# luisdiaz1997/GPzoo

Hardware: AMD Instinct MI355X
Metric: ELBO evals/sec (L=32-latent evaluations, all GPUs) at M=2048 inducing, N=200000, L=32 latents/GPU x 1 GPU(s) (higher is better)
Workload: dtype f32; 1 GPU; BASELINE configs[2]: Slide-seq-shaped synthetic, N=200000 spots, M=2048, L=32 latents/GPU x 1 GPU(s), matern32, f32; latents_total=32, whitened=True, chunk=0, factor_dtype=f64

## Files before the change

gpzoo_amd/_lib.py:

```python
from __future__ import annotations

import ctypes as C
import os

HERE = os.path.dirname(os.path.abspath(__file__))
LIB_PATH = os.environ.get("GPZ_HIP_LIB") or os.path.join(HERE, "libgpzoo_hip.so")

GPZ_F32, GPZ_F64 = 0, 1
KERNEL_RBF, KERNEL_MATERN32, KERNEL_MGGP_RBF, KERNEL_DISTANCE = 0, 1, 2, 3
KERNEL_MATERN12, KERNEL_MATERN52 = 4, 5
SVGP_MATERIALIZE_KZX, SVGP_NARROW_TILES, SVGP_GENERATE_KZX, SVGP_PANEL_PRODUCTS = 1, 2, 4, 8
SVGP_BACKWARD_ALGEBRA, SVGP_BACKWARD_CLASSIC = 16, 32
PROF_SLOTS = ("kfill", "stage1", "stage2", "potrf_trailing", "potrf_all", "trtri", "finalize", "_unused")


class KernelDesc(C.Structure):
    _fields_ = [
        ("kind", C.c_int32), ("n_latent", C.c_int32), ("dtype", C.c_int32), ("n_groups", C.c_int32),
        ("sigma", C.c_void_p), ("lengthscale", C.c_void_p), ("group_a", C.c_void_p), ("group_r2", C.c_void_p),
        ("group_pow", C.c_double),
    ]


class SvgpProblem(C.Structure):
    _fields_ = [
        ("k", KernelDesc),
        ("dtype", C.c_int32), ("whitened", C.c_int32), ("d", C.c_int32), ("flags", C.c_int32),
        ("N", C.c_int64), ("M", C.c_int64),
# ... 147 lines not shown
```

gpzoo_amd/build.py:

```python
from __future__ import annotations

import os
import subprocess
import sys

HERE = os.path.dirname(os.path.abspath(__file__))
CSRC = os.path.join(HERE, "csrc")
LIB = os.path.join(HERE, "libgpzoo_hip.so")
SOURCES = ["runtime.hip", "kfill.hip", "gemm.hip", "gemmw.hip", "gemmp.hip", "diag128.hip", "coop.hip", "factor.hip", "kgrad.hip", "mmops.hip", "poisson.hip", "svgp.hip", "vnngp.hip", "collective.hip", "spatial.hip", "nmf.hip", "smooth.hip", "kmeans.hip", "gram.hip", "poisson_sparse.hip"]
HEADERS = ["common.h", "gemm.h", "cov.h", "gemmw.h", "gemmp.h", "diag128.h", "factor.h", "kgrad.h", "mmops.h", os.path.join("..", "..", "include", "gpzoo_hip.h")]
FLAGS = ["--offload-arch=gfx950", "-O3", "-std=c++17", "-fPIC", "-ffp-contract=fast", "-Wall", "-Wno-unused-function"]
SOURCE_FLAGS = {"spatial.hip": ["-ffp-contract=off"], "smooth.hip": ["-ffp-contract=off"], "kmeans.hip": ["-ffp-contract=off"]}


HASH_MARK = b"GPZ_SRC_HASH:"


def source_hash():
    import hashlib
    h = hashlib.sha256()
    for f in sorted(SOURCES + HEADERS):
        path = os.path.join(CSRC, f)
        if not os.path.exists(path):
            return None
        h.update(os.path.basename(f).encode() + b"\0")
# ... 55 lines not shown
```

gpzoo_amd/csrc/common.h:

```cpp
#pragma once
#include <hip/hip_runtime.h>
#include <stdint.h>
#include <stddef.h>

#include "../../include/gpzoo_hip.h"

namespace gpz {

constexpr int PAD = 128;

inline int64_t pad_up(int64_t v, int64_t m = PAD) { return (v + m - 1) / m * m; }

void set_error(const char* fmt, ...);

#define GPZ_HIP_OK(expr)                                                          \
  do {                                                                            \
    hipError_t _e = (expr);                                                       \
    if (_e != hipSuccess) {                                                       \
      gpz::set_error("%s:%d: %s -> %s", __FILE__, __LINE__, #expr, hipGetErrorString(_e)); \
      return -2;                                                                  \
    }                                                                             \
  } while (0)

#define GPZ_REQUIRE(cond, ...)            \
// ... 14 lines not shown
  template <typename T>
  T* take(size_t count) {
    off = (off + 255) & ~size_t(255);
    T* r = base ? reinterpret_cast<T*>(base + off) : nullptr;
    off += count * sizeof(T);
    return r;
  }
  size_t used() const { return (off + 255) & ~size_t(255); }
};

int kfill_padded(const gpz_kernel_desc* k, const void* A, int64_t nA, int64_t pA, const void* B, int64_t nB,
                 int64_t pB, int d, const int64_t* gA, const int64_t* gB, void* K, int64_t ldk, int64_t stride,
                 double jitter, int pad_identity, int out_dtype, hipStream_t s, int32_t* bad_group = nullptr);

enum ProfSlot { PROF_KFILL = 0, PROF_STAGE1 = 1, PROF_STAGE2 = 2, PROF_POTRF_TRAIL = 3,
                PROF_POTRF_ALL = 4, PROF_TRTRI = 5, PROF_FINAL = 6, PROF_NSLOTS = 8 };
bool prof_enabled();
void prof_begin(int slot, hipStream_t s);
void prof_end(int slot, hipStream_t s);

}
```

gpzoo_amd/csrc/gemmp.h:

```cpp
#pragma once
#include "common.h"

namespace gpz {

struct PanelArgs {
  const float* Linv; const float* LuT;
  const float* Kzx;
  const float* Z; const float* X;
  const float* sigma; const float* ell;
  int64_t M, nreal; int kind, d;
  float* Wt;
  const float* muE;
  float* ps1; float* pm1; float* ps2;
  int64_t Mp, ncp; int L;
};
bool panel_supported(int64_t Mp, int64_t ncp);
bool panel_generates(int kind, int d);
int panel_launch(const PanelArgs& a, hipStream_t s);

}
```

gpzoo_amd/csrc/gemmp.hip:

```cpp
#include "gemmp.h"

#include "cov.h"

#include <cstdlib>
#include <mutex>
#include <type_traits>

#ifndef GPZ_P_ABL
#define GPZ_P_ABL 0
#endif

namespace gpz {

typedef float f32x4 __attribute__((ext_vector_type(4)));
typedef unsigned int u32x4 __attribute__((ext_vector_type(4)));

struct PanelParams {
  const float* Linv; const float* LuT;
  const float* Kzx;
  const float* Z; const float* X;
  const float* sigma; const float* ell;
  int M, nreal;
  float* Wt;
  const float* muE;
// ... 396 lines not shown
      case 6: return launch_t<NBV, 6>(p, store, s);          \
      case 7: return launch_t<NBV, 7>(p, store, s);          \
      case 8: return launch_t<NBV, 8>(p, store, s);          \
      default: return launch_t<NBV, 0>(p, store, s);         \
    }
  switch (a.Mp / 32) {
    GPZ_PANEL_CASE(4)
    GPZ_PANEL_CASE(8)
    GPZ_PANEL_CASE(12)
    default:
    GPZ_PANEL_CASE(16)
  }
#undef GPZ_PANEL_CASE
}

}

extern "C" void gpz_debug_panel_stamps(unsigned long long* buf) { gpz::g_panel_stamps = buf; }
```

gpzoo_amd/csrc/kgrad.hip:

```cpp
#include "kgrad.h"
#include "mmops.h"

namespace gpz {

__device__ __forceinline__ float kg_exp(float x) { return __builtin_amdgcn_exp2f(x * 1.44269504088896341f); }
__device__ __forceinline__ double kg_exp(double x) { return exp(x); }
__device__ __forceinline__ float kg_sqrt(float x) { return sqrtf(x); }
__device__ __forceinline__ double kg_sqrt(double x) { return sqrt(x); }
__device__ __forceinline__ float kg_rsqrt(float x) { return rsqrtf(x); }
__device__ __forceinline__ double kg_rsqrt(double x) { return 1.0 / sqrt(x); }
__device__ __forceinline__ float kg_pow(float x, float y) { return __builtin_amdgcn_exp2f(y * __builtin_amdgcn_logf(x)); }
__device__ __forceinline__ double kg_pow(double x, double y) { return pow(x, y); }

template <typename T, int KIND>
__global__ __launch_bounds__(256) void kgrad_kernel(KgradArgs a) {
  const int l = blockIdx.y, wave = threadIdx.x >> 6, lane = threadIdx.x & 63;
  const int64_t m = (int64_t)blockIdx.x * 4 + wave;
  if (m >= a.M) return;
  const T* kb = static_cast<const T*>(a.Kbar) + (int64_t)l * a.stride + m * a.ld;
  const T* Zp = static_cast<const T*>(a.Z);
  const T* Xp = static_cast<const T*>(a.X);
  const int d = a.d;
  const T sig = static_cast<const T*>(a.sigma)[l];
  const T ell = static_cast<const T*>(a.ell)[l];
  const T s2 = sig * sig, il2 = (T)1 / (ell * ell);
  T z[4] = {0, 0, 0, 0};
  for (int k = 0; k < d; ++k) z[k] = Zp[m * d + k];
  const int gz = (KIND == 2) ? ((uint64_t)a.gZ[m] < (uint64_t)a.G ? (int)a.gZ[m] : 0) : 0;
  const T aeff = (KIND == 2) ? static_cast<const T*>(a.ga)[l] : (T)0;
  const T gpow = (T)a.gpow;
  double dz[4] = {0, 0, 0, 0}, dsig = 0, dell = 0, da = 0;
  constexpr int UN = 4;
  for (int64_t c0 = lane; c0 < a.ncols; c0 += 64 * UN) {
    T g[UN], x[UN][4];
    int gx[UN];
#pragma unroll
    for (int u = 0; u < UN; ++u) {
      const int64_t c = c0 + 64 * u;
      const bool in = c < a.ncols;
      g[u] = in ? kb[c] : (T)0;
#pragma unroll
      for (int k = 0; k < 4; ++k) x[u][k] = (in && k < d) ? Xp[c * d + k] : (T)0;
      gx[u] = (KIND == 2 && in) ? ((uint64_t)a.gX[c] < (uint64_t)a.G ? (int)a.gX[c] : 0) : 0;
    }
    T pz[4] = {0, 0, 0, 0}, psig = 0, pell = 0, pa = 0;
#pragma unroll
    for (int u = 0; u < UN; ++u) {
      T diff[4], d2 = 0;
#pragma unroll
      for (int k = 0; k < 4; ++k) { diff[k] = (k < d) ? z[k] - x[u][k] : (T)0; d2 = fma(diff[k], diff[k], d2); }
      T cz;
      if (KIND == 0) {
        const T kv = s2 * kg_exp((T)-0.5 * d2 * il2);
        psig += g[u] * (T)2 * kv / sig;
        pell += g[u] * kv * d2 * il2 / ell;
        cz = -kv * il2;
      } else if (KIND == 1) {
        const T v = (T)1.7320508075688772935 * kg_sqrt(d2) / ell, e = kg_exp(-v);
        psig += g[u] * (T)2 * sig * ((T)1 + v) * e;
        pell += g[u] * s2 * v * v * e / ell;
        cz = -s2 * (T)3 * il2 * e;
      } else if (KIND == 4) {
        const T rr = kg_sqrt(d2), kv = s2 * kg_exp(-rr / ell);
        psig += g[u] * (T)2 * kv / sig;
        pell += g[u] * kv * rr * il2;
        cz = d2 > (T)0 ? -(kv / ell) * kg_rsqrt(d2) : (T)0;
      } else if (KIND == 5) {
        const T v = (T)2.2360679774997896964 * kg_sqrt(d2) / ell, e = kg_exp(-v), q3 = v * v / (T)3;
        psig += g[u] * (T)2 * sig * ((T)1 + v + q3) * e;
        pell += g[u] * s2 * q3 * ((T)1 + v) * e / ell;
        cz = -s2 * (T)5 / (T)3 * il2 * ((T)1 + v) * e;
      } else {
        const T r2 = static_cast<const T*>(a.gr2)[gz * a.G + gx[u]];
        const T den = aeff * r2 + (T)1;
        const T kv = s2 * kg_exp((T)-0.5 * d2 * il2 / den) * kg_pow(den, -gpow);
        psig += g[u] * (T)2 * kv / sig;
        pell += g[u] * kv * d2 * il2 / (ell * den);
        pa += g[u] * kv * ((T)0.5 * d2 * il2 / (den * den) - gpow / den) * r2;
        cz = -kv * il2 / den;
      }
      const T gc = g[u] * cz;
#pragma unroll
      for (int k = 0; k < 4; ++k) pz[k] = fma(gc, diff[k], pz[k]);
    }
    dsig += (double)psig; dell += (double)pell; da += (double)pa;
#pragma unroll
    for (int k = 0; k < 4; ++k) dz[k] += (double)pz[k];
  }
  double v[7] = {dz[0], dz[1], dz[2], dz[3], dsig * a.scalar_scale, dell * a.scalar_scale, da * a.scalar_scale};
#pragma unroll
  for (int i = 0; i < 7; ++i)
    for (int o = 32; o > 0; o >>= 1) v[i] += __shfl_down(v[i], o);
  if (lane == 0) {
    double* dst = a.acc + ((int64_t)l * a.Mp + m) * 8;
#pragma unroll
    for (int i = 0; i < 7; ++i) dst[i] += v[i];
  }
}

int kgrad_launch(int dtype, int kind, const KgradArgs& a, int L, hipStream_t s) {
  GPZ_REQUIRE((kind >= 0 && kind <= 2) || kind == GPZ_KERNEL_MATERN12 || kind == GPZ_KERNEL_MATERN52,
              "kgrad: unknown kernel kind %d", kind);
  dim3 grid((unsigned)((a.M + 3) / 4), (unsigned)L), block(256);
#define GPZ_KG(T, K) hipLaunchKernelGGL((kgrad_kernel<T, K>), grid, block, 0, s, a)
#define GPZ_KG_KINDS(T) \
  switch (kind) { case 0: GPZ_KG(T, 0); break; case 1: GPZ_KG(T, 1); break; case 4: GPZ_KG(T, 4); break; \
                  case 5: GPZ_KG(T, 5); break; default: GPZ_KG(T, 2); break; }
  if (dtype == GPZ_F32) GPZ_KG_KINDS(float) else GPZ_KG_KINDS(double)
#undef GPZ_KG_KINDS
#undef GPZ_KG
  GPZ_LAUNCH_OK();
  return 0;
}

}

extern "C" size_t gpz_kgrad_workspace_bytes(int64_t nA, int32_t n_latent) {
  if (nA < 1 || n_latent < 1) return 0;
  gpz::Carver c(nullptr);
  c.take<double>((int64_t)n_latent * nA * 8);
  return c.used();
}

extern "C" int gpz_kgrad(const gpz_kernel_desc* k, const void* A, int64_t nA, const void* B, int64_t nB, int32_t d,
                         const int64_t* gA, const int64_t* gB, const void* Kbar, int64_t ldk, int64_t stride_k,
// ... 24 lines not shown
```

gpzoo_amd/csrc/svgp.hip:

```cpp
#include "common.h"
#include "gemmw.h"
#include "gemmp.h"
#include "factor.h"
#include "gemm.h"
#include "kgrad.h"
#include "mmops.h"

#include <algorithm>
#include <cstdlib>
#include <cstring>

namespace gpz {

constexpr int NB = 128;

struct ProductSchedule { int cols, tpw; };
template <typename T>
static ProductSchedule product_schedule(bool stats_epilogue, int nt) {
  const int tpw = (sizeof(T) == 4 && stats_epilogue) ? 2 : 1;
  const int full = 16 * tpw;
  const int strips = (nt + full - 1) / full;
  int w = (nt + strips * tpw - 1) / (strips * tpw);
  if (w > 16) w = 16;
  return ProductSchedule{w * tpw, tpw};
// ... 350 lines not shown

  return 0;
}

static bool panel_path(const gpz_svgp_problem* p, bool f32, int64_t Mp, int64_t ncp) {
  static const int env = [] {
    const char* e = getenv("GPZ_SVGP_PRODUCTS");
    return !e ? 0 : !strcmp(e, "panel") ? 1 : !strcmp(e, "tiles") ? 2 : 0;
  }();
  if (!f32 || !panel_supported(Mp, ncp)) return false;
  if (p->flags & (GPZ_SVGP_NARROW_TILES | GPZ_SVGP_MATERIALIZE_KZX | GPZ_SVGP_GENERATE_KZX)) return false;
  if (p->flags & GPZ_SVGP_PANEL_PRODUCTS) return true;
  return env == 1 || (env == 0 && (panel_generates(p->k.kind, p->d) || Mp >= 256));
}

template <typename T>
static int svgp_forward_t(const gpz_svgp_problem* p, int64_t chunk, void* ws, size_t ws_bytes, hipStream_t s) {
  const Plan pl = make_plan(p, chunk);
  const bool wh = p->whitened != 0;
  Buffers<T> b = carve<T>(pl, wh, ws);
  GPZ_REQUIRE(ws_bytes >= b.bytes, "gpz_svgp_forward: workspace too small (%zu < %zu)", ws_bytes, b.bytes);
  const int64_t L = pl.L, M = pl.M, Mp = pl.Mp, N = pl.N, mm = Mp * Mp;
  const int L32 = (int)L;

  if (int rc = prepare_t<T>(p, pl, b, s)) return rc;

  const int64_t esz = sizeof(T);
  const WtCache<T> wtc = wt_cache_of<T>(pl, p->wt_cache);
  const bool narrow = (p->flags & GPZ_SVGP_NARROW_TILES) != 0;
  const bool fused = !narrow && (p->flags & GPZ_SVGP_GENERATE_KZX) && !(p->flags & GPZ_SVGP_MATERIALIZE_KZX) &&
// ... 407 lines not shown
  const double gk = g_kl[l];
  if (j <= i) {
    const int64_t o = (int64_t)l * Mp * Mp + i * Mp + j;
    G[o] = (T)((double)G[o] + gk * LuW[o]);
  }
  if (j == 0) mu_sum[(int64_t)l * Mp + i] += gk * (double)muE[(int64_t)l * Mp + i];
}

template <typename T>
struct BwdBuffers {
  T *Pc, *H, *G, *G2, *LinvT, *cs; double *mu_part, *mu_sum;
  float* nt_part;
  float* nt_vpart;
  T* gmc;
  T *LuN, *Hd, *GL, *SwI, *csc, *csd, *PS, *A1, *a3; double *D1, *D2, *D3, *D4, *me, *kacc, *sig_direct;
  int32_t* any_d;
  size_t bytes;
};

template <typename T>
static BwdBuffers<T> carve_bwd(const Plan& pl, bool whitened, bool full, void* ws, size_t offset) {
  BwdBuffers<T> b;
  Carver c(ws);
  c.off = offset;
  const int64_t mm = pl.L * pl.Mp * pl.Mp;
  b.Pc = c.take<T>(pl.L * pl.Mp * pl.nc);
  b.H = c.take<T>(mm);
  b.G = c.take<T>(mm);
  b.G2 = whitened ? nullptr : c.take<T>(mm);
  b.LinvT = (whitened && !full) ? nullptr : c.take<T>(mm);
  b.cs = c.take<T>(pl.L * pl.nc);
  b.mu_part = c.take<double>(pl.L * pl.nchunks * pl.Mp);
  b.mu_sum = c.take<double>(pl.L * pl.Mp);
  const size_t ntf = sizeof(T) == 4 && wide_nt_supported(pl.Mp, pl.nc) ? wide_nt_scratch_floats(pl.Mp, pl.nc, (int)pl.L) : 0;
  b.nt_part = ntf ? c.take<float>((int64_t)ntf) : nullptr;
  const bool ntw = sizeof(T) == 4 && wide_nt_supported(pl.Mp, pl.nc);
  b.nt_vpart = ntw ? c.take<float>((int64_t)wide_nt_vpart_floats(pl.Mp, pl.nc, (int)pl.L)) : nullptr;
  b.gmc = c.take<T>(pl.L * pl.nc);
  b.LuN = b.Hd = b.GL = b.SwI = b.csc = b.csd = b.PS = b.A1 = b.a3 = nullptr;
  b.D1 = b.D2 = b.D3 = b.D4 = b.me = b.kacc = b.sig_direct = nullptr;
  b.any_d = nullptr;
  if (full) {
    b.LuN = c.take<T>(mm);
    b.Hd = whitened ? c.take<T>(mm) : nullptr;
    b.PS = c.take<T>(mm);
    b.GL = c.take<T>(mm);
    b.SwI = c.take<T>(mm);
    b.A1 = c.take<T>(mm);
    b.a3 = c.take<T>(pl.L * pl.Mp);
    b.csc = c.take<T>(pl.L * pl.nc);
    b.csd = whitened ? c.take<T>(pl.L * pl.nc) : nullptr;
    b.D1 = c.take<double>(mm);
    b.D2 = c.take<double>(mm);
    b.D3 = c.take<double>(mm);
    b.D4 = whitened ? nullptr : c.take<double>(mm);
    b.me = c.take<double>(pl.L * pl.Mp);
    b.kacc = c.take<double>(pl.L * pl.Mp * 8);
    b.sig_direct = c.take<double>(pl.L);
    b.any_d = c.take<int32_t>(pl.nchunks + 1);
  }
  b.bytes = c.used();
  return b;
}

template <typename TR, typename T>
__global__ __launch_bounds__(256) void q_finish_kernel(TR* __restrict__ R, const T* __restrict__ Hd, int64_t Mp, int64_t M,
                                                      const double* __restrict__ u, const double* __restrict__ v) {
  const int l = blockIdx.z;
  const int64_t i = blockIdx.y, j = (int64_t)blockIdx.x * 256 + threadIdx.x;
  if (j >= Mp || (j >> 7) > (i >> 7)) return;
  const int64_t o = (int64_t)l * Mp * Mp + i * Mp + j;
  double r = (double)R[o];
  if (Hd) r += (double)Hd[o];
  if (i < M && j < M) r += u[(int64_t)l * Mp + i] * v[(int64_t)l * Mp + j];
// ... 194 lines not shown
        g2.super_cols = sched_plain.cols; g2.colscale = w.cs; g2.sCs = ncp; g2.ncols = ncp;
        if (int rc = gemm_launch(g2, EPI_STORE_COLSCALE, s)) return rc;
      }
      if (wide_nt) {
        if constexpr (sizeof(T) == 4) { if (int rc = wide_nt_launch(Wc, w.Pc, w.G, Mp, ncp, L32, s, w.nt_part)) return rc; }
      } else if (int rc = nt_generic(Wc, w.Pc, w.G)) return rc;
    }
    if (!v_done) {
      hipLaunchKernelGGL((rowdot_kernel<T>), dim3((unsigned)(Mp / 4), L32), dim3(256), 0, s, Wc, Mp, ncp,
                         static_cast<const T*>(g->g_mean), N, n0, w.mu_part, pl.nchunks, ci);
      GPZ_LAUNCH_OK();
    }
    if (full) {
      bool done = false;
      if constexpr (sizeof(T) == 4) {
        if (wide && alg) {
          WideArgs wk = {};
          wk.A = w.A1; wk.B = Wc; wk.Mp = Mp; wk.ncp = ncp; wk.L = L32; wk.upper = 2; wk.epilogue = WIDE_KBAR;
          wk.C = w.Pc; wk.colscale = w.cs; wk.colvec = w.gmc; wk.rowvec = w.a3;
          if (int rc = wide_product_launch(wk, s)) return rc;
          if (with_hd) {
            WideArgs wc = {};
            wc.A = w.LinvT; wc.B = Wc; wc.Mp = Mp; wc.ncp = ncp; wc.L = L32; wc.upper = 1; wc.epilogue = WIDE_ADD_COLSCALE;
            wc.C = w.Pc; wc.colscale = w.csd; wc.gate = w.any_d + ci;
            if (int rc = wide_product_launch(wc, s)) return rc;
          }
          done = true;
        }
        if (wide && !alg) {
          WideArgs wa = {};
// ... 344 lines not shown
```

Before: 2.660 ELBO evals/s.

## Fuse Kbar panel product with covariance-gradient reduction in one panel kernel

Adds a panel kernel for the whitened f32 backward pass that computes the Kbar product (A1·W, plus an optional LinvT correction) in registers with MFMA. It then applies the column scaling and immediately accumulates the stationary-kernel gradient sums against Z/X. Per-workgroup partial sums are reduced afterwards, so the dense Kbar panel is never written to memory and re-read by a separate kgrad pass. The kgrad kernel itself is also restructured with vectorised loads and per-dimension specialisation. The cost is a large amount of new complex code and a double-precision partial buffer, with possible numerical differences from the f32 partial accumulation.

```diff
diff --git a/gpzoo_amd/_lib.py b/gpzoo_amd/_lib.py
--- a/gpzoo_amd/_lib.py
+++ b/gpzoo_amd/_lib.py
@@ -11,7 +11,7 @@
 KERNEL_MATERN12, KERNEL_MATERN52 = 4, 5
 SVGP_MATERIALIZE_KZX, SVGP_NARROW_TILES, SVGP_GENERATE_KZX, SVGP_PANEL_PRODUCTS = 1, 2, 4, 8
 SVGP_BACKWARD_ALGEBRA, SVGP_BACKWARD_CLASSIC = 16, 32
-PROF_SLOTS = ("kfill", "stage1", "stage2", "potrf_trailing", "potrf_all", "trtri", "finalize", "_unused")
+PROF_SLOTS = ("kfill", "stage1", "stage2", "potrf_trailing", "potrf_all", "trtri", "finalize", "kbar_panel")
 
 
 class KernelDesc(C.Structure):
diff --git a/gpzoo_amd/build.py b/gpzoo_amd/build.py
--- a/gpzoo_amd/build.py
+++ b/gpzoo_amd/build.py
@@ -8,7 +8,7 @@
 CSRC = os.path.join(HERE, "csrc")
 LIB = os.path.join(HERE, "libgpzoo_hip.so")
 SOURCES = ["runtime.hip", "kfill.hip", "gemm.hip", "gemmw.hip", "gemmp.hip", "diag128.hip", "coop.hip", "factor.hip", "kgrad.hip", "mmops.hip", "poisson.hip", "svgp.hip", "vnngp.hip", "collective.hip", "spatial.hip", "nmf.hip", "smooth.hip", "kmeans.hip", "gram.hip", "poisson_sparse.hip"]
-HEADERS = ["common.h", "gemm.h", "cov.h", "gemmw.h", "gemmp.h", "diag128.h", "factor.h", "kgrad.h", "mmops.h", os.path.join("..", "..", "include", "gpzoo_hip.h")]
+HEADERS = ["common.h", "gemm.h", "cov.h", "covgrad.h", "gemmw.h", "gemmp.h", "diag128.h", "factor.h", "kgrad.h", "mmops.h", os.path.join("..", "..", "include", "gpzoo_hip.h")]
 FLAGS = ["--offload-arch=gfx950", "-O3", "-std=c++17", "-fPIC", "-ffp-contract=fast", "-Wall", "-Wno-unused-function"]
 SOURCE_FLAGS = {"spatial.hip": ["-ffp-contract=off"], "smooth.hip": ["-ffp-contract=off"], "kmeans.hip": ["-ffp-contract=off"]}
 
diff --git a/gpzoo_amd/csrc/common.h b/gpzoo_amd/csrc/common.h
--- a/gpzoo_amd/csrc/common.h
+++ b/gpzoo_amd/csrc/common.h
@@ -52,7 +52,7 @@
                  double jitter, int pad_identity, int out_dtype, hipStream_t s, int32_t* bad_group = nullptr);
 
 enum ProfSlot { PROF_KFILL = 0, PROF_STAGE1 = 1, PROF_STAGE2 = 2, PROF_POTRF_TRAIL = 3,
-                PROF_POTRF_ALL = 4, PROF_TRTRI = 5, PROF_FINAL = 6, PROF_NSLOTS = 8 };
+                PROF_POTRF_ALL = 4, PROF_TRTRI = 5, PROF_FINAL = 6, PROF_KBAR_PANEL = 7, PROF_NSLOTS = 8 };
 bool prof_enabled();
 void prof_begin(int slot, hipStream_t s);
 void prof_end(int slot, hipStream_t s);
diff --git a/gpzoo_amd/csrc/covgrad.h b/gpzoo_amd/csrc/covgrad.h
--- /dev/null
+++ b/gpzoo_amd/csrc/covgrad.h
@@ -0,0 +1,80 @@
+#pragma once
+#include <hip/hip_runtime.h>
+
+namespace gpz {
+
+__device__ __forceinline__ float cg_exp2(float x) { return __builtin_amdgcn_exp2f(x); }
+__device__ __forceinline__ double cg_exp2(double x) { return exp2(x); }
+__device__ __forceinline__ float cg_sqrt(float x) { return __builtin_amdgcn_sqrtf(x); }
+__device__ __forceinline__ double cg_sqrt(double x) { return sqrt(x); }
+__device__ __forceinline__ float cg_rsqrt(float x) { return rsqrtf(x); }
+__device__ __forceinline__ double cg_rsqrt(double x) { return 1.0 / sqrt(x); }
+
+template <typename T> struct CovGradConst { T kex, av; };
+
+template <typename T, int KIND>
+__device__ __forceinline__ CovGradConst<T> covgrad_const(T ell) {
+  const double log2e = 1.44269504088896340736, il = 1.0 / (double)ell;
+  double kex, av = 0.0;
+  if (KIND == 4) kex = -il * log2e;
+  else if (KIND == 5) { av = 2.2360679774997896964 * il; kex = -av * log2e; }
+  else if (KIND == 1) kex = -1.7320508075688772935 * il * log2e;
+  else kex = -0.5 * il * il * log2e;
+  CovGradConst<T> c;
+  c.kex = (T)kex;
+  c.av = (T)av;
+  return c;
+}
+
+template <typename T, int DD> struct CovGradSums {
+  T z[DD], s2, s0, s1;
+  __device__ __forceinline__ void clear() {
+#pragma unroll
+    for (int k = 0; k < DD; ++k) z[k] = (T)0;
+    s2 = s0 = s1 = (T)0;
+  }
+};
+
+template <int KIND, typename T, int DD>
+__device__ __forceinline__ void covgrad_accum(T g, const T (&diff)[DD], T d2, const CovGradConst<T>& c, CovGradSums<T, DD>& s) {
+  T p;
+  if (KIND == 0) {
+    p = g * cg_exp2(c.kex * d2);
+    s.s0 += p;
+  } else if (KIND == 1) {
+    const T r = cg_sqrt(d2);
+    p = g * cg_exp2(c.kex * r);
+    s.s0 += p;
+    s.s1 = fma(p, r, s.s1);
+  } else if (KIND == 5) {
+    const T r = cg_sqrt(d2), ge = g * cg_exp2(c.kex * r);
+    p = fma(c.av * r, ge, ge);
+    s.s0 += p;
+    s.s1 = fma(ge, d2, s.s1);
+  } else {
+    const T ge = g * cg_exp2(c.kex * cg_sqrt(d2));
+    s.s0 += ge;
+    p = d2 > (T)0 ? ge * cg_rsqrt(d2) : (T)0;
+  }
+  s.s2 = fma(p, d2, s.s2);
+#pragma unroll
+  for (int k = 0; k < DD; ++k) s.z[k] = fma(p, diff[k], s.z[k]);
+}
+
+struct CovGradScale { double cz, cl, c0, c1; };
+
+template <int KIND>
+__device__ __forceinline__ CovGradScale covgrad_finish(double sigma, double ell) {
+  const double s2 = sigma * sigma, il = 1.0 / ell;
+  CovGradScale f;
+  f.c0 = 2.0 * sigma;
+  f.c1 = 0.0;
+  if (KIND == 0) { f.cz = -s2 * il * il; }
+  else if (KIND == 1) { f.cz = -3.0 * s2 * il * il; f.c1 = f.c0 * 1.7320508075688772935 * il; }
+  else if (KIND == 5) { f.cz = -(5.0 / 3.0) * s2 * il * il; f.c1 = f.c0 * (5.0 / 3.0) * il * il; }
+  else { f.cz = -s2 * il; }
+  f.cl = -f.cz * il;
+  return f;
+}
+
+}
diff --git a/gpzoo_amd/csrc/gemmp.h b/gpzoo_amd/csrc/gemmp.h
--- a/gpzoo_amd/csrc/gemmp.h
+++ b/gpzoo_amd/csrc/gemmp.h
@@ -18,4 +18,21 @@
 bool panel_generates(int kind, int d);
 int panel_launch(const PanelArgs& a, hipStream_t s);
 
+struct PanelKbarArgs {
+  const float* A1; const float* LinvT;
+  const float* W;
+  const float* cs; const float* gm; const float* csd;
+  const float* a3;
+  const int32_t* any_d;
+  const float* Z; const float* X;
+  const float* sigma; const float* ell;
+  const float* csc; double* sig_direct;
+  int64_t M, nreal; int kind, d;
+  double* part;
+  double* acc;
+  int64_t Mp, ncp; int L;
+};
+size_t panel_kbar_scratch_doubles(int64_t Mp, int64_t ncp, int L);
+int panel_kbar_launch(const PanelKbarArgs& a, hipStream_t s);
+
 }
diff --git a/gpzoo_amd/csrc/gemmp.hip b/gpzoo_amd/csrc/gemmp.hip
--- a/gpzoo_amd/csrc/gemmp.hip
+++ b/gpzoo_amd/csrc/gemmp.hip
@@ -1,6 +1,7 @@
 #include "gemmp.h"
 
 #include "cov.h"
+#include "covgrad.h"
 
 #include <cstdlib>
 #include <mutex>
@@ -434,6 +435,401 @@
 #undef GPZ_PANEL_CASE
 }
 
+constexpr int KB_JOIN = 4, KB_PS = 6;
+
+struct KbarParams {
+  const float* A1; const float* LinvT; const float* W;
+  const float* cs; const float* gm; const float* csd; const float* a3;
+  const int32_t* any_d;
+  const float* Z; const float* X; const float* ell;
+  int M, nreal, Mp, ncp, L, npan, units, nls;
+  double* part;
+};
+
+template <int NB, int KIND, int D>
+__global__ __launch_bounds__(64 * NB) void panel_kbar_kernel(const KbarParams p) {
+  extern __shared__ __attribute__((aligned(16))) float smem[];
+  constexpr int Mp = 32 * NB, PK = Mp + 16, MI = 2, NS = D + 3;
+  float* const P = smem;
+  float* const ex = smem + P_TN * PK;
+  const int tid = threadIdx.x, lane = tid & 63;
+  const int wave = __builtin_amdgcn_readfirstlane(tid >> 6);
+  const int r = lane & 15, q = lane >> 4;
+  const int rb = wave;
+  auto gperm = [](int c) { const int t = (c >> 2) & 3; return (((t >> 1) ^ t) & 1) << 1 | (t >> 1); };
+
+  const int x = blockIdx.x & 7, j = blockIdx.x >> 3, per = gridDim.x >> 3;
+  const int u_lo = (int)((int64_t)x * p.units / 8), u_hi = (int)((int64_t)(x + 1) * p.units / 8);
+  if (u_lo + j >= u_hi) return;
+  const int l_first = (u_lo + j) / p.npan;
+
+  int a_voff[MI];
+#pragma unroll
+  for (int mi = 0; mi < MI; ++mi) a_voff[mi] = ((rb * 32 + mi * 16 + r) * Mp + 4 * q) * 4;
+  const float* const bfrag = P + r * PK + ((q ^ gperm(r)) << 2);
+  const int kd = rb * 32;
+
+  constexpr int NR = 8, RP = 4 * NB;
+  f32x4 pv[NR];
+  const int pc4 = tid & 15, pk_of = tid >> 4;
+  auto panel_fetch = [&](int l, int64_t col0, auto lo_c, auto hi_c) __attribute__((always_inline)) {
+#if defined(__HIP_DEVICE_COMPILE__)
+    const __amdgpu_buffer_rsrc_t kr = __builtin_amdgcn_make_buffer_rsrc(
+        const_cast<float*>(p.W + (int64_t)l * Mp * p.ncp + col0), 0, (Mp - 1) * p.ncp * 4 + P_TN * 4, 0x00020000);
+    const int voff = (pk_of * p.ncp + 4 * pc4) * 4, sstep = RP * p.ncp * 4;
+#pragma unroll
+    for (int i = decltype(lo_c)::value; i < decltype(hi_c)::value; ++i)
+      pv[i] = __builtin_bit_cast(f32x4, __builtin_amdgcn_raw_buffer_load_b128(kr, voff, i * sstep, 0));
+#endif
+  };
+  auto panel_next = [&](int ln, int64_t coln, auto lo_c, auto hi_c) __attribute__((always_inline)) {
+    if (ln >= 0) panel_fetch(ln, coln, lo_c, hi_c);
+    else {
+#pragma unroll
+      for (int i = decltype(lo_c)::value; i < decltype(hi_c)::value; ++i) pv[i] = f32x4{0, 0, 0, 0};
+    }
+  };
+  auto panel_write = [&]() __attribute__((always_inline)) {
+    int kof = pk_of;
+    asm volatile("" : "+v"(kof));
+#pragma unroll
+    for (int i = 0; i < NR; ++i) {
+      const int k = i * RP + kof;
+#pragma unroll
+      for (int e = 0; e < 4; ++e) {
+        const int c = 4 * pc4 + e;
+        P[c * PK + (k & ~15) + ((((k >> 2) & 3) ^ gperm(c)) << 2) + (k & 3)] = pv[i][e];
+      }
+    }
+  };
+
+  f32x4 acc[MI][4];
+  f32x4 fa0[MI], fb0[4], fa1[MI], fb1[4];
+  float sB[4] = {1.f, 1.f, 1.f, 1.f};
+  using std::integral_constant;
+  using i0 = integral_constant<int, 0>;
+  using i4 = integral_constant<int, 4>;
+  using i6 = integral_constant<int, 6>;
+  using i8 = integral_constant<int, 8>;
+  auto mma = [&](const f32x4 (&fa)[MI], const f32x4 (&fb)[4], auto scaled_c) __attribute__((always_inline)) {
+    constexpr bool SCALED = decltype(scaled_c)::value != 0;
+#pragma unroll
+    for (int jj = 0; jj < 4; ++jj)
+#pragma unroll
+      for (int ni = 0; ni < 4; ++ni) {
+        const float b = SCALED ? fb[ni][jj] * sB[ni] : fb[ni][jj];
+#pragma unroll
+        for (int mi = 0; mi < MI; ++mi)
+          acc[mi][ni] = __builtin_amdgcn_mfma_f32_16x16x4f32(b, fa[mi][jj], acc[mi][ni], 0, 0, 0);
+      }
+    __builtin_amdgcn_sched_barrier(0);
+  };
+  auto load_a = [&](const float* A, int l, f32x4 (&fa)[MI], int k0) __attribute__((always_inline)) {
+#if defined(__HIP_DEVICE_COMPILE__)
+    if (GPZ_P_ABL & 4) return;
+    const __amdgpu_buffer_rsrc_t ar = __builtin_amdgcn_make_buffer_rsrc(
+        const_cast<float*>(A + (int64_t)l * Mp * Mp), 0, Mp * Mp * 4, 0x00020000);
+#pragma unroll
+    for (int mi = 0; mi < MI; ++mi)
+      fa[mi] = __builtin_bit_cast(f32x4, __builtin_amdgcn_raw_buffer_load_b128(ar, a_voff[mi], k0 * 4, 0));
+#endif
+  };
+  auto load_b = [&](f32x4 (&fb)[4], int k0) __attribute__((always_inline)) {
+    if (GPZ_P_ABL & 8) return;
+#pragma unroll
+    for (int ni = 0; ni < 4; ++ni) fb[ni] = *reinterpret_cast<const f32x4*>(bfrag + ni * 16 * PK + k0);
+  };
+  auto load = [&](const float* A, int l, f32x4 (&fa)[MI], f32x4 (&fb)[4], int k0) __attribute__((always_inline)) {
+    load_a(A, l, fa, k0);
+    load_b(fb, k0);
+    __builtin_amdgcn_sched_barrier(0);
+  };
+  auto product = [&](const float* A, int l, int k0, auto scaled_c) __attribute__((always_inline)) {
+    load_b(fb0, k0);
+    __builtin_amdgcn_sched_barrier(0);
+#pragma unroll 1
+    for (int k = k0; k < Mp; k += 32) {
+      load(A, l, fa1, fb1, k + 16);
+      mma(fa0, fb0, scaled_c);
+      if (k + 32 < Mp) load(A, l, fa0, fb0, k + 32);
+      mma(fa1, fb1, scaled_c);
+    }
+  };
+
+  float z[MI][D];
+#pragma unroll
+  for (int mi = 0; mi < MI; ++mi) {
+    const int m = rb * 32 + mi * 16 + r;
+#pragma unroll
+    for (int k = 0; k < D; ++k) z[mi][k] = m < p.M ? p.Z[m * D + k] : 0.f;
+  }
+  CovGradSums<float, D> ps[MI];
+#pragma unroll
+  for (int mi = 0; mi < MI; ++mi) ps[mi].clear();
+  bool fresh = true;
+  int since = 0;
+  auto flush = [&](int l) __attribute__((always_inline)) {
+    const int slot = l - l_first;
+#pragma unroll
+    for (int mi = 0; mi < MI; ++mi) {
+      float v[NS];
+#pragma unroll
+      for (int k = 0; k < D; ++k) v[k] = ps[mi].z[k];
+      v[D] = ps[mi].s2; v[D + 1] = ps[mi].s0; v[D + 2] = ps[mi].s1;
+#pragma unroll
+      for (int i = 0; i < NS; ++i) { v[i] += __shfl_xor(v[i], 16); v[i] += __shfl_xor(v[i], 32); }
+      if (q == 0 && slot < p.nls) {
+        double* dst = p.part + (((int64_t)blockIdx.x * p.nls + slot) * Mp + rb * 32 + mi * 16 + r) * KB_PS;
+#pragma unroll
+        for (int i = 0; i < NS; ++i) dst[i] = (fresh ? 0.0 : dst[i]) + (double)v[i];
+      }
+      ps[mi].clear();
+    }
+    fresh = false;
+    since = 0;
+  };
+
+  const int any = p.any_d ? __builtin_amdgcn_readfirstlane(*p.any_d) : 0;
+  int u = u_lo + j;
+  int l = u / p.npan, pn = u - l * p.npan;
+  panel_fetch(l, (int64_t)pn * P_TN, i0{}, i8{});
+#pragma unroll 1
+  for (;;) {
+    const int64_t col0 = (int64_t)pn * P_TN;
+    const int un = u + per;
+    load_a(p.A1, l, fa0, 0);
+    const CovGradConst<float> cc = covgrad_const<float, KIND>(p.ell[l]);
+    float a3r[MI];
+#pragma unroll
+    for (int mi = 0; mi < MI; ++mi) a3r[mi] = p.a3[(int64_t)l * Mp + rb * 32 + mi * 16 + r];
+    __builtin_amdgcn_sched_barrier(0);
+    panel_write();
+    if (tid < 64) {
+      const int64_t n = col0 + tid;
+      const bool real = n < p.nreal;
+#pragma unroll
+      for (int k = 0; k < D; ++k) ex[k * 64 + tid] = real ? p.X[n * D + k] : 0.f;
+      ex[2 * 64 + tid] = p.cs[(int64_t)l * p.ncp + n];
+      ex[3 * 64 + tid] = p.gm[(int64_t)l * p.ncp + n];
+      ex[4 * 64 + tid] = p.csd ? p.csd[(int64_t)l * p.ncp + n] : 0.f;
+    }
+    __syncthreads();
+
+#pragma unroll
+    for (int mi = 0; mi < MI; ++mi)
+#pragma unroll
+      for (int ni = 0; ni < 4; ++ni) acc[mi][ni] = f32x4{0, 0, 0, 0};
+    product(p.A1, l, 0, i0{});
+    {
+#pragma unroll
+      for (int ni = 0; ni < 4; ++ni) {
+        const f32x4 c4 = *reinterpret_cast<const f32x4*>(ex + 2 * 64 + ni * 16 + 4 * q);
+        const f32x4 g4 = *reinterpret_cast<const f32x4*>(ex + 3 * 64 + ni * 16 + 4 * q);
+#pragma unroll
+        for (int mi = 0; mi < MI; ++mi)
+#pragma unroll
+          for (int g = 0; g < 4; ++g) acc[mi][ni][g] = __builtin_fmaf(a3r[mi], g4[g], acc[mi][ni][g] * c4[g]);
+      }
+    }
+    if (any) {
+#pragma unroll
+      for (int ni = 0; ni < 4; ++ni) sB[ni] = ex[4 * 64 + ni * 16 + r];
+      load_a(p.LinvT, l, fa0, kd);
+      __builtin_amdgcn_sched_barrier(0);
+      product(p.LinvT, l, kd, integral_constant<int, 1>{});
+    }
+    const int ln = un < u_hi ? un / p.npan : -1;
+    const int64_t coln = (int64_t)(un - ln * p.npan) * P_TN;
+    panel_next(ln, coln, i0{}, i4{});
+    __builtin_amdgcn_sched_barrier(0);
+    if (GPZ_P_ABL & 16) {
+#pragma unroll
+      for (int mi = 0; mi < MI; ++mi)
+#pragma unroll
+        for (int ni = 0; ni < 4; ++ni) asm volatile("" ::"v"(acc[mi][ni]));
+      panel_next(ln, coln, i4{}, i8{});
+    } else {
+#pragma unroll
+      for (int ni = 0; ni < 4; ++ni) {
+        f32x4 xc[D];
+#pragma unroll
+        for (int k = 0; k < D; ++k) xc[k] = *reinterpret_cast<const f32x4*>(ex + k * 64 + ni * 16 + 4 * q);
+#pragma unroll
+        for (int g = 0; g < 4; ++g)
+#pragma unroll
+          for (int mi = 0; mi < MI; ++mi) {
+            float diff[D], d2 = 0.f;
+#pragma unroll
+            for (int k = 0; k < D; ++k) { diff[k] = z[mi][k] - xc[k][g]; d2 = __builtin_fmaf(diff[k], diff[k], d2); }
+            covgrad_accum<KIND>(acc[mi][ni][g], diff, d2, cc, ps[mi]);
+          }
+#pragma unroll
+        for (int mi = 0; mi < MI; ++mi) {
+#pragma unroll
+          for (int k = 0; k < D; ++k) asm volatile("" : "+v"(ps[mi].z[k]));
+          asm volatile("" : "+v"(ps[mi].s2), "+v"(ps[mi].s0), "+v"(ps[mi].s1));
+        }
+        __builtin_amdgcn_sched_barrier(0);
+        if (ni == 0) panel_next(ln, coln, i4{}, i6{});
+        if (ni == 1) panel_next(ln, coln, i6{}, i8{});
+        __builtin_amdgcn_sched_barrier(0);
+      }
+    }
+    ++since;
+    if (ln != l) { flush(l); fresh = true; }
+    else if (since == KB_JOIN) flush(l);
+    __syncthreads();
+    if (un >= u_hi) break;
+    u = un; pn = un - ln * p.npan; l = ln;
+  }
+}
+
+struct KbarReduceParams {
+  const double* part; double* acc; const float* sigma; const float* ell;
+  const float* csc; double* sig_direct;
+  int M, Mp, ncp, L, npan, units, nls, wgs, d;
+};
+
+constexpr int KBR_R = 4;
+template <int KIND>
+__global__ __launch_bounds__(256) void panel_kbar_reduce_kernel(const KbarReduceParams a) {
+  __shared__ double sh[256][KBR_R * 5];
+  __shared__ double tot[KBR_R * 5];
+  __shared__ double sd[4];
+  const int l = blockIdx.y, row0 = blockIdx.x * KBR_R, tid = threadIdx.x;
+  const int per = a.wgs >> 3, ns = a.d + 3;
+  double t = 0.0;
+  for (int base = 0; base < a.wgs; base += 256) {
+    const int wg = base + tid;
+    const double* src = nullptr;
+    if (wg < a.wgs) {
+      const int x = wg & 7, j = wg >> 3;
+      const int u_lo = (int)((int64_t)x * a.units / 8), u_hi = (int)((int64_t)(x + 1) * a.units / 8);
+      const int u0 = u_lo + j;
+      if (u0 < u_hi) {
+        const int lo = l * a.npan, hi = (l + 1) * a.npan < u_hi ? (l + 1) * a.npan : u_hi;
+        const int u = lo > u0 ? u0 + (lo - u0 + per - 1) / per * per : u0;
+        const int slot = l - u0 / a.npan;
+        if (u < hi && slot >= 0 && slot < a.nls) src = a.part + (((int64_t)wg * a.nls + slot) * a.Mp + row0) * KB_PS;
+      }
+    }
+#pragma unroll
+    for (int r = 0; r < KBR_R; ++r)
+#pragma unroll
+      for (int i = 0; i < 5; ++i) sh[tid][r * 5 + i] = (src && i < ns && row0 + r < a.Mp) ? src[r * KB_PS + i] : 0.0;
+    __syncthreads();
+    if (tid < KBR_R * 5)
+      for (int w = 0; w < 256; ++w) t += sh[w][tid];
+    __syncthreads();
+  }
+  if (tid < KBR_R * 5) tot[tid] = t;
+  __syncthreads();
+  if (tid < KBR_R && row0 + tid < a.M) {
+    const double* v = tot + tid * 5;
+    const CovGradScale f = covgrad_finish<KIND>((double)a.sigma[l], (double)a.ell[l]);
+    double* dst = a.acc + ((int64_t)l * a.Mp + row0 + tid) * 8;
+    for (int k = 0; k < a.d; ++k) dst[k] += f.cz * v[k];
+    dst[4] += f.c0 * v[a.d + 1] + f.c1 * v[a.d + 2];
+    dst[5] += f.cl * v[a.d];
+  }
+  if (blockIdx.x == 0) {
+    double c = 0.0;
+    for (int64_t n = tid; n < a.ncp; n += 256) c += (double)a.csc[(int64_t)l * a.ncp + n];
+    for (int o = 32; o > 0; o >>= 1) c += __shfl_down(c, o);
+    if ((tid & 63) == 0) sd[tid >> 6] = c;
+    __syncthreads();
+    if (tid == 0) a.sig_direct[l] += (double)a.sigma[l] * (((sd[0] + sd[1]) + sd[2]) + sd[3]);
+  }
+}
+
+static int kbar_nls(int L) { return L / 8 + 2 < L ? L / 8 + 2 : L; }
+static int kbar_max_wgs(int64_t ncp, int L) {
+  const int64_t units8 = (L * (ncp / P_TN) + 7) / 8 * 8;
+  return (int)(units8 < 512 ? units8 : 512);
+}
+
+size_t panel_kbar_scratch_doubles(int64_t Mp, int64_t ncp, int L) {
+  return (size_t)kbar_max_wgs(ncp, L) * kbar_nls(L) * Mp * KB_PS;
+}
+
+template <int NB, int KIND, int D>
+static int kbar_launch_t(const KbarParams& p, hipStream_t s, int* wgs_out) {
+  const size_t lds = sizeof(float) * ((size_t)P_TN * (p.Mp + 16) + 5 * 64);
+  struct PerDevice { bool attr = false; int cus = 0; };
+  static PerDevice seen[64];
+  static std::mutex mu;
+  int dev = 0;
+  GPZ_HIP_OK(hipGetDevice(&dev));
+  int cus = 256;
+  {
+    std::lock_guard<std::mutex> lock(mu);
+    PerDevice& d = seen[dev & 63];
+    if (!d.attr) {
+      GPZ_HIP_OK(hipFuncSetAttribute(reinterpret_cast<const void*>(&panel_kbar_kernel<NB, KIND, D>),
+                                     hipFuncAttributeMaxDynamicSharedMemorySize, (int)lds));
+      int n = 0;
+      if (hipDeviceGetAttribute(&n, hipDeviceAttributeMultiprocessorCount, dev) != hipSuccess || n < 8) n = 256;
+      d.cus = n;
+      d.attr = true;
+    }
+    cus = d.cus;
+  }
+  const int per_cu = (int)((160 * 1024) / lds) < 1 ? 1 : (int)((160 * 1024) / lds);
+  int wgs = cus * (per_cu > 2 ? 2 : per_cu);
+  wgs -= wgs % 8;
+  const int cap = kbar_max_wgs(p.ncp, p.L);
+  if (wgs > cap) wgs = cap;
+  *wgs_out = wgs;
+  hipLaunchKernelGGL((panel_kbar_kernel<NB, KIND, D>), dim3(wgs), dim3(64 * NB), lds, s, p);
+  GPZ_LAUNCH_OK();
+  return 0;
+}
+
+template <int KIND, int D>
+static int kbar_launch_nb(const KbarParams& p, hipStream_t s, int* wgs) {
+  switch (p.Mp / 32) {
+    case 4: return kbar_launch_t<4, KIND, D>(p, s, wgs);
+    case 8: return kbar_launch_t<8, KIND, D>(p, s, wgs);
+    case 12: return kbar_launch_t<12, KIND, D>(p, s, wgs);
+    default: return kbar_launch_t<16, KIND, D>(p, s, wgs);
+  }
+}
+
+int panel_kbar_launch(const PanelKbarArgs& a, hipStream_t s) {
+  GPZ_REQUIRE(panel_supported(a.Mp, a.ncp) && panel_generates(a.kind, a.d), "panel_kbar_launch: unsupported Mp=%lld ncp=%lld kind=%d d=%d",
+              (long long)a.Mp, (long long)a.ncp, a.kind, a.d);
+  GPZ_REQUIRE(a.A1 && a.W && a.cs && a.gm && a.a3 && a.Z && a.X && a.sigma && a.ell && a.csc && a.sig_direct && a.part && a.acc &&
+              a.M >= 1 && a.M <= a.Mp && a.nreal >= 1 && a.nreal <= a.ncp && (!a.any_d || (a.LinvT && a.csd)),
+              "panel_kbar_launch: bad arguments");
+  KbarParams p = {};
+  p.A1 = a.A1; p.LinvT = a.LinvT; p.W = a.W; p.cs = a.cs; p.gm = a.gm; p.csd = a.csd; p.a3 = a.a3; p.any_d = a.any_d;
+  p.Z = a.Z; p.X = a.X; p.ell = a.ell; p.M = (int)a.M; p.nreal = (int)a.nreal; p.Mp = (int)a.Mp; p.ncp = (int)a.ncp;
+  p.L = a.L; p.npan = (int)(a.ncp / P_TN); p.units = a.L * p.npan; p.nls = kbar_nls(a.L); p.part = a.part;
+  int wgs = 0, rc = 0;
+#define GPZ_KBAR_KIND(K) (a.d == 1 ? kbar_launch_nb<K, 1>(p, s, &wgs) : kbar_launch_nb<K, 2>(p, s, &wgs))
+  switch (a.kind) {
+    case GPZ_KERNEL_RBF: rc = GPZ_KBAR_KIND(0); break;
+    case GPZ_KERNEL_MATERN32: rc = GPZ_KBAR_KIND(1); break;
+    case GPZ_KERNEL_MATERN12: rc = GPZ_KBAR_KIND(4); break;
+    default: rc = GPZ_KBAR_KIND(5); break;
+  }
+#undef GPZ_KBAR_KIND
+  if (rc) return rc;
+  KbarReduceParams q = {};
+  q.part = a.part; q.acc = a.acc; q.sigma = a.sigma; q.ell = a.ell; q.csc = a.csc; q.sig_direct = a.sig_direct;
+  q.M = (int)a.M; q.Mp = (int)a.Mp; q.ncp = (int)a.ncp; q.L = a.L; q.npan = p.npan; q.units = p.units; q.nls = p.nls;
+  q.wgs = wgs; q.d = a.d;
+  const dim3 grid((unsigned)((a.M + KBR_R - 1) / KBR_R), (unsigned)a.L);
+  switch (a.kind) {
+    case GPZ_KERNEL_RBF: hipLaunchKernelGGL(panel_kbar_reduce_kernel<0>, grid, dim3(256), 0, s, q); break;
+    case GPZ_KERNEL_MATERN32: hipLaunchKernelGGL(panel_kbar_reduce_kernel<1>, grid, dim3(256), 0, s, q); break;
+    case GPZ_KERNEL_MATERN12: hipLaunchKernelGGL(panel_kbar_reduce_kernel<4>, grid, dim3(256), 0, s, q); break;
+    default: hipLaunchKernelGGL(panel_kbar_reduce_kernel<5>, grid, dim3(256), 0, s, q); break;
+  }
+  GPZ_LAUNCH_OK();
+  return 0;
+}
+
 }
 
 extern "C" void gpz_debug_panel_stamps(unsigned long long* buf) { gpz::g_panel_stamps = buf; }
diff --git a/gpzoo_amd/csrc/kgrad.hip b/gpzoo_amd/csrc/kgrad.hip
--- a/gpzoo_amd/csrc/kgrad.hip
+++ b/gpzoo_amd/csrc/kgrad.hip
@@ -1,4 +1,5 @@
 #include "kgrad.h"
+#include "covgrad.h"
 #include "mmops.h"
 
 namespace gpz {
@@ -12,8 +13,8 @@
 __device__ __forceinline__ float kg_pow(float x, float y) { return __builtin_amdgcn_exp2f(y * __builtin_amdgcn_logf(x)); }
 __device__ __forceinline__ double kg_pow(double x, double y) { return pow(x, y); }
 
-template <typename T, int KIND>
-__global__ __launch_bounds__(256) void kgrad_kernel(KgradArgs a) {
+template <typename T>
+__global__ __launch_bounds__(256) void kgrad_mggp_kernel(KgradArgs a) {
   const int l = blockIdx.y, wave = threadIdx.x >> 6, lane = threadIdx.x & 63;
   const int64_t m = (int64_t)blockIdx.x * 4 + wave;
   if (m >= a.M) return;
@@ -26,8 +27,8 @@
   const T s2 = sig * sig, il2 = (T)1 / (ell * ell);
   T z[4] = {0, 0, 0, 0};
   for (int k = 0; k < d; ++k) z[k] = Zp[m * d + k];
-  const int gz = (KIND == 2) ? ((uint64_t)a.gZ[m] < (uint64_t)a.G ? (int)a.gZ[m] : 0) : 0;
-  const T aeff = (KIND == 2) ? static_cast<const T*>(a.ga)[l] : (T)0;
+  const int gz = (uint64_t)a.gZ[m] < (uint64_t)a.G ? (int)a.gZ[m] : 0;
+  const T aeff = static_cast<const T*>(a.ga)[l];
   const T gpow = (T)a.gpow;
   double dz[4] = {0, 0, 0, 0}, dsig = 0, dell = 0, da = 0;
   constexpr int UN = 4;
@@ -41,7 +42,7 @@
       g[u] = in ? kb[c] : (T)0;
 #pragma unroll
       for (int k = 0; k < 4; ++k) x[u][k] = (in && k < d) ? Xp[c * d + k] : (T)0;
-      gx[u] = (KIND == 2 && in) ? ((uint64_t)a.gX[c] < (uint64_t)a.G ? (int)a.gX[c] : 0) : 0;
+      gx[u] = in ? ((uint64_t)a.gX[c] < (uint64_t)a.G ? (int)a.gX[c] : 0) : 0;
     }
     T pz[4] = {0, 0, 0, 0}, psig = 0, pell = 0, pa = 0;
 #pragma unroll
@@ -49,37 +50,13 @@
       T diff[4], d2 = 0;
 #pragma unroll
       for (int k = 0; k < 4; ++k) { diff[k] = (k < d) ? z[k] - x[u][k] : (T)0; d2 = fma(diff[k], diff[k], d2); }
-      T cz;
-      if (KIND == 0) {
-        const T kv = s2 * kg_exp((T)-0.5 * d2 * il2);
-        psig += g[u] * (T)2 * kv / sig;
-        pell += g[u] * kv * d2 * il2 / ell;
-        cz = -kv * il2;
-      } else if (KIND == 1) {
-        const T v = (T)1.7320508075688772935 * kg_sqrt(d2) / ell, e = kg_exp(-v);
-        psig += g[u] * (T)2 * sig * ((T)1 + v) * e;
-        pell += g[u] * s2 * v * v * e / ell;
-        cz = -s2 * (T)3 * il2 * e;
-      } else if (KIND == 4) {
-        const T rr = kg_sqrt(d2), kv = s2 * kg_exp(-rr / ell);
-        psig += g[u] * (T)2 * kv / sig;
-        pell += g[u] * kv * rr * il2;
-        cz = d2 > (T)0 ? -(kv / ell) * kg_rsqrt(d2) : (T)0;
-      } else if (KIND == 5) {
-        const T v = (T)2.2360679774997896964 * kg_sqrt(d2) / ell, e = kg_exp(-v), q3 = v * v / (T)3;
-        psig += g[u] * (T)2 * sig * ((T)1 + v + q3) * e;
-        pell += g[u] * s2 * q3 * ((T)1 + v) * e / ell;
-        cz = -s2 * (T)5 / (T)3 * il2 * ((T)1 + v) * e;
-      } else {
-        const T r2 = static_cast<const T*>(a.gr2)[gz * a.G + gx[u]];
-        const T den = aeff * r2 + (T)1;
-        const T kv = s2 * kg_exp((T)-0.5 * d2 * il2 / den) * kg_pow(den, -gpow);
-        psig += g[u] * (T)2 * kv / sig;
-        pell += g[u] * kv * d2 * il2 / (ell * den);
-        pa += g[u] * kv * ((T)0.5 * d2 * il2 / (den * den) - gpow / den) * r2;
-        cz = -kv * il2 / den;
-      }
-      const T gc = g[u] * cz;
+      const T r2 = static_cast<const T*>(a.gr2)[gz * a.G + gx[u]];
+      const T den = aeff * r2 + (T)1;
+      const T kv = s2 * kg_exp((T)-0.5 * d2 * il2 / den) * kg_pow(den, -gpow);
+      psig += g[u] * (T)2 * kv / sig;
+      pell += g[u] * kv * d2 * il2 / (ell * den);
+      pa += g[u] * kv * ((T)0.5 * d2 * il2 / (den * den) - gpow / den) * r2;
+      const T gc = g[u] * (-kv * il2 / den);
 #pragma unroll
       for (int k = 0; k < 4; ++k) pz[k] = fma(gc, diff[k], pz[k]);
     }
@@ -98,17 +75,166 @@
   }
 }
 
+constexpr int KG_RW = 4, KG_JOIN = 4;
+
+template <typename T, int KIND, int ND, bool VEC>
+__global__ __launch_bounds__(256) void kgrad_kernel(KgradArgs a) {
+  constexpr int DD = ND ? ND : 4, NS = DD + 3;
+  typedef T vec4 __attribute__((ext_vector_type(4)));
+  __shared__ double sh[4][KG_RW][NS];
+  const int l = blockIdx.y, wave = threadIdx.x >> 6, lane = threadIdx.x & 63;
+  const int64_t m0 = (int64_t)blockIdx.x * KG_RW;
+  const int d = ND ? ND : a.d;
+  const T* Zp = static_cast<const T*>(a.Z);
+  const T* Xp = static_cast<const T*>(a.X);
+  const CovGradConst<T> cc = covgrad_const<T, KIND>(static_cast<const T*>(a.ell)[l]);
+  const T* kb[KG_RW];
+  T z[KG_RW][DD], keep[KG_RW];
+#pragma unroll
+  for (int r = 0; r < KG_RW; ++r) {
+    const bool ok = m0 + r < a.M;
+    const int64_t m = ok ? m0 + r : a.M - 1;
+    keep[r] = ok ? (T)1 : (T)0;
+    kb[r] = static_cast<const T*>(a.Kbar) + (int64_t)l * a.stride + m * a.ld;
+#pragma unroll
+    for (int k = 0; k < DD; ++k) z[r][k] = k < d ? Zp[m * d + k] : (T)0;
+  }
+  const int64_t nsteps = (a.ncols + 255) / 256;
+
+  auto load = [&](int64_t s, T (&g)[KG_RW][4], T (&x)[4][DD]) __attribute__((always_inline)) {
+    const int64_t base = s * 256;
+    if (VEC && base + 256 <= a.ncols) {
+      const int64_t c = base + 4 * lane;
+#pragma unroll
+      for (int r = 0; r < KG_RW; ++r) {
+        const vec4 v = *reinterpret_cast<const vec4*>(kb[r] + c);
+#pragma unroll
+        for (int u = 0; u < 4; ++u) g[r][u] = v[u];
+      }
+      if constexpr (ND == 1) {
+        const vec4 v = *reinterpret_cast<const vec4*>(Xp + c);
+#pragma unroll
+        for (int u = 0; u < 4; ++u) x[u][0] = v[u];
+      } else if constexpr (ND == 2) {
+        const vec4 v0 = *reinterpret_cast<const vec4*>(Xp + 2 * c), v1 = *reinterpret_cast<const vec4*>(Xp + 2 * c + 4);
+        x[0][0] = v0[0]; x[0][1] = v0[1]; x[1][0] = v0[2]; x[1][1] = v0[3];
+        x[2][0] = v1[0]; x[2][1] = v1[1]; x[3][0] = v1[2]; x[3][1] = v1[3];
+      } else {
+#pragma unroll
+        for (int u = 0; u < 4; ++u)
+#pragma unroll
+          for (int k = 0; k < DD; ++k) x[u][k] = k < d ? Xp[(c + u) * d + k] : (T)0;
+      }
+    } else {
+#pragma unroll
+      for (int u = 0; u < 4; ++u) {
+        const int64_t c = base + lane + 64 * u;
+        const bool in = c < a.ncols;
+#pragma unroll
+        for (int r = 0; r < KG_RW; ++r) g[r][u] = in ? kb[r][c] : (T)0;
+#pragma unroll
+        for (int k = 0; k < DD; ++k) x[u][k] = (in && k < d) ? Xp[c * d + k] : (T)0;
+      }
+    }
+  };
+
+  CovGradSums<T, DD> ps[KG_RW];
+  double tot[KG_RW][NS];
+#pragma unroll
+  for (int r = 0; r < KG_RW; ++r) {
+    ps[r].clear();
+#pragma unroll
+    for (int i = 0; i < NS; ++i) tot[r][i] = 0.0;
+  }
+  auto join = [&]() __attribute__((always_inline)) {
+#pragma unroll
+    for (int r = 0; r < KG_RW; ++r) {
+#pragma unroll
+      for (int k = 0; k < DD; ++k) tot[r][k] += (double)ps[r].z[k];
+      tot[r][DD] += (double)ps[r].s2; tot[r][DD + 1] += (double)ps[r].s0; tot[r][DD + 2] += (double)ps[r].s1;
+      ps[r].clear();
+    }
+  };
+  int since = 0;
+  auto step = [&](const T (&g)[KG_RW][4], const T (&x)[4][DD]) __attribute__((always_inline)) {
+#pragma unroll
+    for (int u = 0; u < 4; ++u)
+#pragma unroll
+      for (int r = 0; r < KG_RW; ++r) {
+        T diff[DD], d2 = (T)0;
+#pragma unroll
+        for (int k = 0; k < DD; ++k) { diff[k] = z[r][k] - x[u][k]; d2 = fma(diff[k], diff[k], d2); }
+        covgrad_accum<KIND>(g[r][u] * keep[r], diff, d2, cc, ps[r]);
+      }
+    if (++since == KG_JOIN) { join(); since = 0; }
+  };
+
+  T g0[KG_RW][4], x0[4][DD], g1[KG_RW][4], x1[4][DD];
+  int64_t s = wave;
+  if (s < nsteps) {
+    load(s, g0, x0);
+#pragma unroll 1
+    for (;;) {
+      const bool more1 = s + 4 < nsteps;
+      if (more1) load(s + 4, g1, x1);
+      step(g0, x0);
+      if (!more1) break;
+      const bool more0 = s + 8 < nsteps;
+      if (more0) load(s + 8, g0, x0);
+      step(g1, x1);
+      if (!more0) break;
+      s += 8;
+    }
+    join();
+  }
+#pragma unroll
+  for (int r = 0; r < KG_RW; ++r)
+#pragma unroll
+    for (int i = 0; i < NS; ++i) {
+      double v = tot[r][i];
+      for (int o = 32; o > 0; o >>= 1) v += __shfl_down(v, o);
+      if (lane == 0) sh[wave][r][i] = v;
+    }
+  __syncthreads();
+  if (threadIdx.x < KG_RW && m0 + threadIdx.x < a.M) {
+    const int r = threadIdx.x;
+    double v[NS];
+#pragma unroll
+    for (int i = 0; i < NS; ++i) v[i] = ((sh[0][r][i] + sh[1][r][i]) + sh[2][r][i]) + sh[3][r][i];
+    const CovGradScale f = covgrad_finish<KIND>((double)static_cast<const T*>(a.sigma)[l], (double)static_cast<const T*>(a.ell)[l]);
+    double* dst = a.acc + ((int64_t)l * a.Mp + m0 + r) * 8;
+#pragma unroll
+    for (int k = 0; k < DD; ++k)
+      if (k < d) dst[k] += f.cz * v[k];
+    dst[4] += (f.c0 * v[DD + 1] + f.c1 * v[DD + 2]) * a.scalar_scale;
+    dst[5] += f.cl * v[DD] * a.scalar_scale;
+  }
+}
+
+template <typename T, int KIND>
+static void kgrad_stationary(const KgradArgs& a, int L, hipStream_t s) {
+  const uintptr_t al = 4 * sizeof(T);
+  const bool vec = reinterpret_cast<uintptr_t>(a.Kbar) % al == 0 && reinterpret_cast<uintptr_t>(a.X) % al == 0 &&
+                   a.ld % 4 == 0 && a.stride % 4 == 0;
+  dim3 grid((unsigned)((a.M + KG_RW - 1) / KG_RW), (unsigned)L), block(256);
+#define GPZ_KG(ND, V) hipLaunchKernelGGL((kgrad_kernel<T, KIND, ND, V>), grid, block, 0, s, a)
+#define GPZ_KG_D(V) \
+  switch (a.d) { case 1: GPZ_KG(1, V); break; case 2: GPZ_KG(2, V); break; default: GPZ_KG(0, V); break; }
+  if (vec) GPZ_KG_D(true) else GPZ_KG_D(false)
+#undef GPZ_KG_D
+#undef GPZ_KG
+}
+
 int kgrad_launch(int dtype, int kind, const KgradArgs& a, int L, hipStream_t s) {
   GPZ_REQUIRE((kind >= 0 && kind <= 2) || kind == GPZ_KERNEL_MATERN12 || kind == GPZ_KERNEL_MATERN52,
               "kgrad: unknown kernel kind %d", kind);
-  dim3 grid((unsigned)((a.M + 3) / 4), (unsigned)L), block(256);
-#define GPZ_KG(T, K) hipLaunchKernelGGL((kgrad_kernel<T, K>), grid, block, 0, s, a)
+  GPZ_REQUIRE(a.d >= 1 && a.d <= 4 && a.M >= 1, "kgrad: bad extents d=%d M=%lld", a.d, (long long)a.M);
 #define GPZ_KG_KINDS(T) \
-  switch (kind) { case 0: GPZ_KG(T, 0); break; case 1: GPZ_KG(T, 1); break; case 4: GPZ_KG(T, 4); break; \
-                  case 5: GPZ_KG(T, 5); break; default: GPZ_KG(T, 2); break; }
+  switch (kind) { case 0: kgrad_stationary<T, 0>(a, L, s); break; case 1: kgrad_stationary<T, 1>(a, L, s); break; \
+                  case 4: kgrad_stationary<T, 4>(a, L, s); break; case 5: kgrad_stationary<T, 5>(a, L, s); break; \
+                  default: hipLaunchKernelGGL((kgrad_mggp_kernel<T>), dim3((unsigned)((a.M + 3) / 4), (unsigned)L), dim3(256), 0, s, a); break; }
   if (dtype == GPZ_F32) GPZ_KG_KINDS(float) else GPZ_KG_KINDS(double)
 #undef GPZ_KG_KINDS
-#undef GPZ_KG
   GPZ_LAUNCH_OK();
   return 0;
 }
diff --git a/gpzoo_amd/csrc/svgp.hip b/gpzoo_amd/csrc/svgp.hip
--- a/gpzoo_amd/csrc/svgp.hip
+++ b/gpzoo_amd/csrc/svgp.hip
@@ -388,6 +388,15 @@
   return env == 1 || (env == 0 && (panel_generates(p->k.kind, p->d) || Mp >= 256));
 }
 
+static bool kbar_panel_path(const gpz_svgp_problem* p, bool f32, int64_t Mp, int64_t ncp) {
+  static const int env = [] {
+    const char* e = getenv("GPZ_SVGP_KBAR");
+    return !e ? 0 : !strcmp(e, "panel") ? 1 : !strcmp(e, "tiles") ? 2 : 0;
+  }();
+  if (!f32 || !panel_supported(Mp, ncp) || !panel_generates(p->k.kind, p->d)) return false;
+  return env != 2;
+}
+
 template <typename T>
 static int svgp_forward_t(const gpz_svgp_problem* p, int64_t chunk, void* ws, size_t ws_bytes, hipStream_t s) {
   const Plan pl = make_plan(p, chunk);
@@ -825,6 +834,7 @@
   float* nt_vpart;
   T* gmc;
   T *LuN, *Hd, *GL, *SwI, *csc, *csd, *PS, *A1, *a3; double *D1, *D2, *D3, *D4, *me, *kacc, *sig_direct;
+  double* kpart;
   int32_t* any_d;
   size_t bytes;
 };
@@ -851,6 +861,7 @@
   b.LuN = b.Hd = b.GL = b.SwI = b.csc = b.csd = b.PS = b.A1 = b.a3 = nullptr;
   b.D1 = b.D2 = b.D3 = b.D4 = b.me = b.kacc = b.sig_direct = nullptr;
   b.any_d = nullptr;
+  b.kpart = nullptr;
   if (full) {
     b.LuN = c.take<T>(mm);
     b.Hd = whitened ? c.take<T>(mm) : nullptr;
@@ -869,6 +880,7 @@
     b.kacc = c.take<double>(pl.L * pl.Mp * 8);
     b.sig_direct = c.take<double>(pl.L);
     b.any_d = c.take<int32_t>(pl.nchunks + 1);
+    if (sizeof(T) == 4 && panel_supported(pl.Mp, pl.nc)) b.kpart = c.take<double>(panel_kbar_scratch_doubles(pl.Mp, pl.nc, (int)pl.L));
   }
   b.bytes = c.used();
   return b;
@@ -1093,6 +1105,21 @@
     if (full) {
       bool done = false;
       if constexpr (sizeof(T) == 4) {
+        if (wide && alg && w.kpart && kbar_panel_path(p, pl.f32, Mp, ncp)) {
+          PanelKbarArgs ka = {};
+          ka.A1 = (const float*)w.A1; ka.W = (const float*)Wc; ka.cs = (const float*)w.cs; ka.gm = (const float*)w.gmc;
+          ka.a3 = (const float*)w.a3;
+          if (with_hd) { ka.LinvT = (const float*)w.LinvT; ka.csd = (const float*)w.csd; ka.any_d = w.any_d + ci; }
+          ka.Z = static_cast<const float*>(p->Z); ka.X = static_cast<const float*>(Xc);
+          ka.sigma = static_cast<const float*>(p->k.sigma); ka.ell = static_cast<const float*>(p->k.lengthscale);
+          ka.csc = (const float*)w.csc; ka.sig_direct = w.sig_direct;
+          ka.M = M; ka.nreal = nreal; ka.kind = p->k.kind; ka.d = p->d; ka.part = w.kpart; ka.acc = w.kacc;
+          ka.Mp = Mp; ka.ncp = ncp; ka.L = L32;
+          prof_begin(PROF_KBAR_PANEL, s);
+          if (int rc = panel_kbar_launch(ka, s)) return rc;
+          prof_end(PROF_KBAR_PANEL, s);
+          continue;
+        }
         if (wide && alg) {
           WideArgs wk = {};
           wk.A = w.A1; wk.B = Wc; wk.Mp = Mp; wk.ncp = ncp; wk.L = L32; wk.upper = 2; wk.epilogue = WIDE_KBAR;
```

Result: no change. 2.662 ELBO evals/s, median of 6 (+0.1%).
